# marella/ctransformers

Measured on NVIDIA H100. Metric: decode tokens/s Llama-2-7B Q4_K_M b=1, higher is better.
Workload: dtype int8 (q4_K/q6_K weights x q8_K activations, mma.sync u8 x s8 -> exact int32), fp32 combine in the reference's order

## Files before the change

ctransformers_b200/csrc/matvec.cuh:

```cuda
#pragma once
#include "device_types.cuh"
#include "attention.cuh"

namespace ctb {

#ifndef CTB_THREADS
#define CTB_THREADS 512
#endif
constexpr int MV_THREADS = CTB_THREADS;
constexpr int MV_WARPS = MV_THREADS / 32;
constexpr int MV_ROWS = 4;
constexpr int MV_MAX_SEG = 3;

enum : int { NORM_NONE = 0, NORM_RMS = 1, NORM_LAYER = 2 };
enum : int { EPI_STORE = 0, EPI_ADD = 1, EPI_GELU = 2, EPI_ADD2 = 3, EPI_SILU = 4 };

#ifndef ST_WATCHDOG_NS
#define ST_WATCHDOG_NS 4000000000ull
#endif
#ifndef XC_WATCHDOG_NS
#define XC_WATCHDOG_NS 30000000000ull
#endif
enum WaitCode : int {
  W_GRID_BARRIER = 1, W_FOLD_FLAG, W_FREE_WEIGHT_SLOT, W_WEIGHT_ITEM, W_FREE_K_SLOT, W_FREE_V_SLOT, W_K_ITEM, W_V_ITEM, W_XCHG,
// ... 78 lines not shown

template <bool CG = false>
__device__ __forceinline__ void load16(const float* p, int valid, float (&v)[16]) {
  if (valid >= 16) {
    float4 a, b, c, d;
    if (CG) { a = __ldcg((const float4*)p); b = __ldcg((const float4*)p + 1); c = __ldcg((const float4*)p + 2); d = __ldcg((const float4*)p + 3); }
    else { a = __ldg((const float4*)p); b = __ldg((const float4*)p + 1); c = __ldg((const float4*)p + 2); d = __ldg((const float4*)p + 3); }
    v[0] = a.x; v[1] = a.y; v[2] = a.z; v[3] = a.w; v[4] = b.x; v[5] = b.y; v[6] = b.z; v[7] = b.w;
    v[8] = c.x; v[9] = c.y; v[10] = c.z; v[11] = c.w; v[12] = d.x; v[13] = d.y; v[14] = d.z; v[15] = d.w;
  } else {
#pragma unroll
    for (int e = 0; e < 16; e++) v[e] = e < valid ? (CG ? __ldcg(p + e) : __ldg(p + e)) : 0.f;
  }
}

template <int NT, int BAR>
__device__ __forceinline__ double block_sum_f64(double s, double* red ) {
  s = warp_sum(s);
  bar_sync<BAR, NT>();
  if ((threadIdx.x & 31) == 0) red[threadIdx.x >> 5] = s;
  bar_sync<BAR, NT>();
  double t = 0.0;
#pragma unroll
  for (int w = 0; w < NT / 32; w++) t += red[w];
  return t;
}
template <int NT, int BAR>
__device__ __forceinline__ void block_sum2_max_f64(double& s, double& a, double& g, double* red) {
  constexpr int NW = NT / 32;
#pragma unroll
  for (int o = 16; o > 0; o >>= 1) {
    s += __shfl_xor_sync(0xffffffffu, s, o);
    a += __shfl_xor_sync(0xffffffffu, a, o);
    g = fmax(g, __shfl_xor_sync(0xffffffffu, g, o));
  }
  bar_sync<BAR, NT>();
  if ((threadIdx.x & 31) == 0) { red[threadIdx.x >> 5] = s; red[NW + (threadIdx.x >> 5)] = a; red[2 * NW + (threadIdx.x >> 5)] = g; }
  bar_sync<BAR, NT>();
  s = 0.0;
  a = 0.0;
#pragma unroll
  for (int w = 0; w < NW; w++) { s += red[w]; a += red[NW + w]; g = fmax(g, red[2 * NW + w]); }
}

__device__ __forceinline__ uint32_t pack4(const int* q) {
  return (uint32_t)(q[0] & 0xff) | ((uint32_t)(q[1] & 0xff) << 8) | ((uint32_t)(q[2] & 0xff) << 16) | ((uint32_t)(q[3] & 0xff) << 24);
}

__device__ __forceinline__ void load16_ll(const uint2* p, unsigned epoch, float (&u)[16]) {
  uint4 q[8];
  bounded_wait([&] {
// ... 77 lines not shown
                                           unsigned epoch) {
  const int K = xs.K;
  if (a_is_s) a = s = block_sum_f64<NT, BAR>(s, red);
  else block_sum2_max_f64<NT, BAR>(s, a, g, red);
  if (!isfinite(s) || (!a_is_s && __dmul_ru(a, g) < 0x1p52)) return (float)(s / (double)K);
  const double e = __dmul_ru(a, (double)K * 0x1.0000001p-52);
  const float lo = (float)(__dsub_rd(s, e) / (double)K), hi = (float)(__dadd_ru(s, e) / (double)K);
  if (lo == hi) return lo;
  const double seq = threadIdx.x < 32 ? seq_sum_warp0<XC>(xs.x, xs.x2, xs.x_mode, xs.x_parts, xs.x_stride, K, kind, mean, epoch) : 0.0;
  bar_sync<BAR, NT>();
  if (threadIdx.x == 0) red[0] = seq;
  bar_sync<BAR, NT>();
  return (float)(red[0] / (double)K);
}

template <int NT, int BAR, bool XC = false>
__device__ __forceinline__ void stage_activation(const MVParams& xs, const NormPre& np, int act, uint8_t* smem, double* red, bool write_norm, unsigned epoch = 0) {
  const float* nw = xs.norm_w;
  const float* nb_ = xs.norm_b;
  float* norm_out = xs.norm_out;
  const int norm_mode = xs.norm_mode, K = xs.K;
  const float eps = xs.eps;
  const int t = threadIdx.x, lane = t & 31;
  const int passes = (K + NT * 16 - 1) / (NT * 16);
  float mean = 0.f, scale = 1.f;
  float v0[16];
  load16x<XC>(xs, t * 16, K - t * 16, v0, epoch);
  if (norm_mode == NORM_RMS) {
    double ss = 0.0;
    for (int ps = 0; ps < passes; ps++) {
      const int base = (ps * NT + t) * 16;
      if ((base & ~511) >= K) continue;
// ... 20 lines not shown
        s1 += (double)v[e];
        a1 += (double)fabsf(v[e]);
        emin = min_exp(emin, v[e]);
      }
    }
    mean = norm_stat<NT, BAR, XC>(s1, a1, lsb_inv(emin), false, NORM_TERM_X, 0.f, xs, red, epoch);
    double s2 = 0.0;
    for (int ps = 0; ps < passes; ps++) {
      const int base = (ps * NT + t) * 16;
      if ((base & ~511) >= K) continue;
      float v[16];
      load16x<XC>(xs, base, K - base, v, epoch);
#pragma unroll
      for (int e = 0; e < 16; e++) { const float d = (base + e < K) ? __fsub_rn(v[e], mean) : 0.f; s2 += (double)__fmul_rn(d, d); }
    }
    const float var = norm_stat<NT, BAR, XC>(s2, s2, 0.0, true, NORM_TERM_DEV, mean, xs, red, epoch);
    scale = __fdiv_rn(1.0f, __fsqrt_rn(__fadd_rn(var, eps)));
  }
  int8_t* qs = (int8_t*)smem;
  const size_t off = ((size_t)K + 15) & ~(size_t)15;
  float* dd = (float*)(smem + off);
  int16_t* bs = (int16_t*)(smem + off + q8k_d_bytes(K));
  for (int ps = 0; ps < passes; ps++) {
    const int base = (ps * NT + t) * 16;
    const int valid = K - base;
    if ((base & ~511) >= K) continue;
    float v[16];
    if (ps == 0) {
#pragma unroll
      for (int e = 0; e < 16; e++) v[e] = v0[e];
    } else load16x<XC>(xs, base, valid, v, epoch);
// ... 23 lines not shown
    if (write_norm && norm_out && valid > 0) {
#pragma unroll
      for (int e = 0; e < 16; e++) if (e < valid) norm_out[base + e] = v[e];
    }
    if (act == ACT_Q8_K) {
      float amax = 0.f, mx = 0.f;
#pragma unroll
      for (int e = 0; e < 16; e++) { const float ax = fabsf(v[e]); if (ax > amax) { amax = ax; mx = v[e]; } }
      float gmax = amax;
#pragma unroll
      for (int o = 8; o > 0; o >>= 1) gmax = fmaxf(gmax, __shfl_xor_sync(0xffffffffu, gmax, o));
      const unsigned who = __ballot_sync(0xffffffffu, amax == gmax);
      const int hbase = lane & 16, hl = lane & 15;
      const unsigned mine = (who >> hbase) & 0xffffu;
      const float maxv = __shfl_sync(0xffffffffu, mx, hbase + __ffs(mine) - 1);
      if (valid > 0) {
        const int b = base >> 8;
        int q[16];
        int sum = 0;
        if (gmax == 0.f) {
#pragma unroll
          for (int e = 0; e < 16; e++) q[e] = 0;
          if (hl == 0) dd[b] = 0.f;
        } else {
          const float iscale = __fdiv_rn(-128.f, maxv);
#pragma unroll
          for (int e = 0; e < 16; e++) {
            const float val = __fmaf_rn(iscale, v[e], 12582912.f);
            q[e] = min(127, (__float_as_int(val) & 0x007fffff) - 0x00400000);
            sum += q[e];
          }
          if (hl == 0) dd[b] = __fdiv_rn(1.f, iscale);
        }
        bs[b * 16 + hl] = (int16_t)sum;
#pragma unroll
        for (int j = 0; j < 4; j++) {
          const int wi = hl * 4 + j;
          *(uint32_t*)(qs + q8k_word_offset(b, wi >> 3, wi & 7)) = pack4(q + 4 * j);
        }
      }
    } else if (act == ACT_Q8_0) {
      float amax = 0.f;
#pragma unroll
      for (int e = 0; e < 16; e++) amax = fmaxf(amax, fabsf(v[e]));
      amax = fmaxf(amax, __shfl_xor_sync(0xffffffffu, amax, 1));
      if (valid > 0) {
        const float d = __fdiv_rn(amax, 127.f);
        const float id = amax != 0.f ? __fdiv_rn(127.f, amax) : 0.f;
        int q[16];
#pragma unroll
        for (int e = 0; e < 16; e++) q[e] = __float2int_rn(__fmul_rn(v[e], id));
        *(uint4*)(qs + base) = make_uint4(pack4(q), pack4(q + 4), pack4(q + 8), pack4(q + 12));
        if ((lane & 1) == 0) dd[base >> 5] = h2f(f2h(d));
      }
// ... 156 lines not shown
__device__ __forceinline__ float table_f16(const uint16_t* tab, float x) { return h2f(__ldg(tab + f2h(x))); }

__device__ __forceinline__ float epilogue(int epi, float v, const float* res, const float* res2, const MVParams& p) {
  if (epi == EPI_ADD) return __fadd_rn(v, __ldcg(res));
  if (epi == EPI_ADD2) return __fadd_rn(__fadd_rn(v, __ldcg(res)), __ldcg(res2));
  if (epi == EPI_GELU) return table_f16(p.gelu_tab, v);
  if (epi == EPI_SILU) return table_f16(p.silu_tab, v);
  return v;
}
__device__ __forceinline__ void store_epilogue(const MVSeg& sg, const MVParams& p, int row, float v) { sg.out[row] = epilogue(sg.epi, v, sg.res + row, sg.res2 + row, p); }

__host__ __device__ inline int rows_per_unit(int type) { return (type == GT_F16 || type == GT_F32) ? 1 : MV_ROWS; }

static __global__ void __launch_bounds__(MV_THREADS, 1) k_matvec(const __grid_constant__ MVParams p) {
  extern __shared__ __align__(16) uint8_t smem[];
  __shared__ double red[3 * MV_WARPS];
  const int warp = threadIdx.x >> 5, lane = threadIdx.x & 31;
  pdl_trigger();
  NormPre np;
  preload_norm(np, p);
  pdl_wait();
  stage_activation<MV_THREADS, 0>(p, np, p.act, smem, red, blockIdx.x == 0);
  const ActView a = act_view(p.act, p.K, smem);
  const int gw = blockIdx.x * MV_WARPS + warp, nw = gridDim.x * MV_WARPS;
  int first = gw;
  for (int s = 0; s < p.nseg; s++) {
    const MVSeg& sg = p.seg[s];
    const int type = sg.w.type;
    const int rpu = rows_per_unit(type);
    const int units = (sg.w.M + rpu - 1) / rpu;
    int un = first;
// ... 34 lines not shown
```

ctransformers_b200/csrc/ops_abi.cu:

```cuda
#include <cmath>
#include <cstdio>
#include <cstring>
#include <functional>
#include <memory>
#include <stdexcept>
#include <string>
#include <vector>

#include "../../include/ctransformers_b200.h"
#include "attention.cuh"
#include "matvec.cuh"
#include "prefill.cuh"
#include "repack.cuh"
#include "stream.cuh"
#include "tables.hpp"

using namespace ctb;

namespace {

#define OPS_CUDA(expr)                                                                                     \
  do {                                                                                                     \
    cudaError_t e__ = (expr);                                                                              \
    if (e__ != cudaSuccess) throw std::runtime_error(std::string("CUDA error: ") + cudaGetErrorString(e__) + " (" #expr ")"); \
// ... 69 lines not shown
  o.m.qs = (const uint8_t*)pl[0]; o.m.qh = (const uint8_t*)pl[1]; o.m.d = pl[2]; o.m.mn = pl[3];
}

int sm_count() {
  int n_sm = 132;
  cudaDeviceGetAttribute(&n_sm, cudaDevAttrMultiProcessorCount, 0);
  return n_sm;
}

unsigned* sync_words() {
  static unsigned* d_sync = nullptr;
  if (!d_sync) { OPS_CUDA(cudaMalloc((void**)&d_sync, 64)); OPS_CUDA(cudaMemset(d_sync, 0, 64)); }
  return d_sync;
}

void run_phases(std::vector<Phase> phs) {
  unsigned* d_sync = sync_words();
  const StepLaunch L = step_launch_shape(phs.data(), (int)phs.size(), sm_count(), max_dyn_smem(k_step<true, false>));
  const std::vector<int> hb = step_bounds(phs.data(), (int)phs.size(), L.grid);
  DevBuf dbounds(hb.size() * 4);
  OPS_CUDA(cudaMemcpy(dbounds.p, hb.data(), hb.size() * 4, cudaMemcpyHostToDevice));
  if (L.n_slots < ST_W) throw std::runtime_error("rows too long for the step kernel's shared memory");
  OPS_CUDA(step_set_smem_limit(L.smem));
  DevBuf dprog((phs.size() + 1) * sizeof(Phase));
  OPS_CUDA(cudaMemcpy(dprog.p, phs.data(), phs.size() * sizeof(Phase), cudaMemcpyHostToDevice));
  OPS_CUDA(launch_step(L, 0, dprog.as<Phase>(), dbounds.as<int>(), (int)phs.size(), d_sync));
  OPS_CUDA(cudaGetLastError());
  OPS_CUDA(cudaDeviceSynchronize());
}

void run_matvec(MVParams& p) {
  p.silu_tab = tables().silu;
  p.gelu_tab = tables().gelu;
  if (step_supports(p)) {
    run_phases({matvec_phase(p)});
    return;
  }
  static bool attr = false;
  if (!attr) {
    OPS_CUDA(matvec_set_smem_limit(MV_SMEM_LIMIT));
    attr = true;
  }
  const MVLaunch L = matvec_launch_shape(p, sm_count());
  OPS_CUDA(launch_matvec_kernel(L, 0, p));
  OPS_CUDA(cudaGetLastError());
}

__global__ void __launch_bounds__(MV_THREADS) k_stage_dump(const __grid_constant__ MVParams q, int act, uint8_t* dump) {
  extern __shared__ __align__(16) uint8_t smem[];
  __shared__ double red[3 * MV_WARPS];
  NormPre np;
  preload_norm(np, q);
  stage_activation<MV_THREADS, 0>(q, np, act, smem, red, true);
  const size_t n = act_smem_bytes(act, q.K);
  for (size_t i = threadIdx.x; i < n; i += MV_THREADS) dump[i] = smem[i];
}

__global__ void __launch_bounds__(MV_THREADS) k_gate_dump(const __grid_constant__ MVParams q, float* out) {
  extern __shared__ __align__(16) uint8_t smem[];
  __shared__ double red[3 * MV_WARPS];
  NormPre np;
  preload_norm(np, q);
  stage_activation<MV_THREADS, 0>(q, np, ACT_F32, smem, red, false);
  const float* f = (const float*)smem;
  for (int i = threadIdx.x; i < q.K; i += MV_THREADS) out[i] = f[i];
}

__global__ void k_rope_dump(float* x, const float2* rope, int pos, int hd, int neox) {
  float* row = x + (size_t)blockIdx.x * hd;
  int i0, i1;
  float o0, o1;
  rope_head_pair(row, threadIdx.x, hd, neox, rope[(size_t)pos * (hd / 2) + threadIdx.x], i0, i1, o0, o1);
  row[i0] = o0; row[i1] = o1;
}

int guarded(const char* what, const std::function<void()>& fn) {
  try {
    int ndev = 0;
    if (cudaGetDeviceCount(&ndev) != cudaSuccess || ndev == 0) throw std::runtime_error("no CUDA device available (no CPU fallback)");
    fn();
    return 0;
  } catch (const std::exception& e) {
    fprintf(stderr, "ctransformers-b200: %s failed: %s\n", what, e.what());
    return -1;
  }
}

void stage_to_host(const float* x, const float* w, const float* b, float* y_norm, int mode, float eps, int K, int act, std::vector<uint8_t>& dump) {
  DevBuf dx((size_t)K * 4), dw((size_t)K * 4), db((size_t)K * 4), dy((size_t)K * 4);
  OPS_CUDA(cudaMemcpy(dx.p, x, (size_t)K * 4, cudaMemcpyHostToDevice));
  if (w) OPS_CUDA(cudaMemcpy(dw.p, w, (size_t)K * 4, cudaMemcpyHostToDevice));
  if (b) OPS_CUDA(cudaMemcpy(db.p, b, (size_t)K * 4, cudaMemcpyHostToDevice));
  const size_t n = act_smem_bytes(act, K);
  DevBuf dd(n);
  if (n > 48 * 1024) OPS_CUDA(cudaFuncSetAttribute(k_stage_dump, cudaFuncAttributeMaxDynamicSharedMemorySize, (int)n));
  MVParams q{};
  q.x = dx.as<float>(); q.norm_w = w ? dw.as<float>() : nullptr; q.norm_b = b ? db.as<float>() : nullptr; q.norm_out = dy.as<float>();
  q.norm_mode = mode; q.eps = eps; q.K = K;
  k_stage_dump<<<1, MV_THREADS, n>>>(q, act, dd.as<uint8_t>());
// ... 36 lines not shown
    for (int n = 0; n < N; n++) {
      MVParams p{};
      p.x = dx.as<float>() + (size_t)n * K; p.norm_mode = NORM_NONE; p.K = K; p.act = act_format_for(type); p.nseg = 1;
      p.seg[0].w = w.m; p.seg[0].out = dy.as<float>() + (size_t)n * M; p.seg[0].epi = EPI_STORE;
      run_matvec(p);
    }
    OPS_CUDA(cudaMemcpy(dst, dy.p, (size_t)M * N * 4, cudaMemcpyDeviceToHost));
  });
}

int ctb_quantize_row_q8_K(const float* x, void* y, int k) {
  return guarded("ctb_quantize_row_q8_K", [&] {
    if (k % 256) throw std::runtime_error("k must be a multiple of 256");
    std::vector<uint8_t> dump;
    stage_to_host(x, nullptr, nullptr, nullptr, NORM_NONE, 0.f, k, ACT_Q8_K, dump);
    const int nb = k / 256;
    const size_t off = ((size_t)k + 15) & ~(size_t)15;
    const float* d = (const float*)(dump.data() + off);
    const int16_t* bs = (const int16_t*)(dump.data() + off + q8k_d_bytes(k));
    uint8_t* out = (uint8_t*)y;
    for (int b = 0; b < nb; b++) {
      memcpy(out + (size_t)b * 292, d + b, 4);
      for (int e = 0; e < 256; e++) {
        const int wd = e >> 2, sb = wd >> 3, ln = wd & 7;
        out[(size_t)b * 292 + 4 + e] = dump[(size_t)((b * 2 + (sb >> 2)) * 8 + ln) * 16 + (sb & 3) * 4 + (e & 3)];
      }
      memcpy(out + (size_t)b * 292 + 260, bs + (size_t)b * 16, 32);
    }
  });
}

int ctb_quantize_row_q8_0(const float* x, void* y, int k) {
  return guarded("ctb_quantize_row_q8_0", [&] {
    if (k % 32) throw std::runtime_error("k must be a multiple of 32");
    std::vector<uint8_t> dump;
    stage_to_host(x, nullptr, nullptr, nullptr, NORM_NONE, 0.f, k, ACT_Q8_0, dump);
    const int nb = k / 32;
    const size_t off = ((size_t)k + 15) & ~(size_t)15;
    const float* d = (const float*)(dump.data() + off);
    uint8_t* out = (uint8_t*)y;
    for (int b = 0; b < nb; b++) {
      const uint16_t h = __half_as_ushort(__float2half_rn(d[b]));
      memcpy(out + (size_t)b * 34, &h, 2);
// ... 35 lines not shown
    if (n < 256 || n % 256) throw std::runtime_error("the step kernel takes n a positive multiple of 256");
    const std::vector<uint8_t> zeros(raw_row_bytes(GT_Q4_K, n) * 16, 0);
    OwnedMat wm;
    upload(wm, GT_Q4_K, zeros.data(), n, 16);
    DevBuf dx((size_t)n * 4), dw((size_t)n * 4), db((size_t)n * 4), dy((size_t)n * 4), dout(16 * 4);
    OPS_CUDA(cudaMemcpy(dx.p, x, (size_t)n * 4, cudaMemcpyHostToDevice));
    if (w) OPS_CUDA(cudaMemcpy(dw.p, w, (size_t)n * 4, cudaMemcpyHostToDevice));
    if (b) OPS_CUDA(cudaMemcpy(db.p, b, (size_t)n * 4, cudaMemcpyHostToDevice));
    MVParams p{};
    p.x = dx.as<float>(); p.norm_w = w ? dw.as<float>() : nullptr; p.norm_b = b && mode == NORM_LAYER ? db.as<float>() : nullptr;
    p.norm_out = dy.as<float>(); p.norm_mode = mode; p.eps = eps; p.K = n; p.act = ACT_Q8_K; p.nseg = 1;
    p.seg[0].w = wm.m; p.seg[0].out = dout.as<float>(); p.seg[0].epi = EPI_STORE;
    p.silu_tab = tables().silu; p.gelu_tab = tables().gelu;
    run_phases({matvec_phase(p)});
    OPS_CUDA(cudaMemcpy(y, dy.p, (size_t)n * 4, cudaMemcpyDeviceToHost));
  });
}

int ctb_rope(float* x, int n_heads, int head_dim, int pos, int mode, float freq_base, float freq_scale) {
  return guarded("ctb_rope", [&] {
    const int half = head_dim / 2;
    const std::vector<float2> tab = rope_table(pos + 1, head_dim, head_dim, freq_base, freq_scale);
    const size_t nq = (size_t)n_heads * head_dim;
    DevBuf dq(nq * 4), dtab(tab.size() * 8);
    OPS_CUDA(cudaMemcpy(dq.p, x, nq * 4, cudaMemcpyHostToDevice));
    OPS_CUDA(cudaMemcpy(dtab.p, tab.data(), tab.size() * 8, cudaMemcpyHostToDevice));
    k_rope_dump<<<n_heads, half>>>(dq.as<float>(), dtab.as<float2>(), pos, head_dim, (mode & 2) ? 1 : 0);
    OPS_CUDA(cudaGetLastError());
    OPS_CUDA(cudaMemcpy(x, dq.p, nq * 4, cudaMemcpyDeviceToHost));
  });
// ... 261 lines not shown
```

ctransformers_b200/csrc/prefill.cuh:

```cuda
#pragma once
#include "stream.cuh"

namespace ctb {

constexpr int PB_T = 32;
constexpr int PB_TG = PB_T / 8;
constexpr int PB_TEAMS = 2;
constexpr int PB_W = PB_TEAMS * 4;
constexpr int PB_NT = PB_W * 32;
constexpr int PB_THREADS = PB_NT + 32;
constexpr int PB_BAR = 1;
constexpr int PB_XCH = 12 * 16 * PB_T * 4;

enum : int { PP_EMBED = 0, PP_QUANT = 1, PP_GEMM = 2, PP_KV = 3, PP_ATTN = 4 };

__host__ __device__ inline size_t pb_qbuf_bytes(int K) { return (size_t)(K / 256) * (8192 + 512 + 128); }

struct alignas(16) PPhase {
  int kind;
  MVParams mv;
  int x_ld, x2_ld;
  int out_ld[MV_MAX_SEG], res_ld[MV_MAX_SEG], res2_ld[MV_MAX_SEG];
  uint8_t* qbuf;
  AttnParams at;
// ... 319 lines not shown
__device__ __forceinline__ void pb_attn_phase(const PPhase& ph, int n_tok, uint8_t* work) {
  const int warp = threadIdx.x >> 5;
  const int n_tasks = n_tok * ph.at.n_head;
  uint8_t* wsm = work + (size_t)warp * pb_attn_warp_bytes(ph.at.n_ctx, ph.at.hd);
  for (int task = blockIdx.x * PB_W + warp; task < n_tasks; task += (int)gridDim.x * PB_W) {
    const int tok = task / ph.at.n_head;
    pb_attn_warp_task<GEN>(ph.at, ph.state + tok * 4, tok, task % ph.at.n_head, wsm);
  }
}
static __device__ __noinline__ void pb_attn_phase_gen(const PPhase& ph, int n_tok, uint8_t* work) { pb_attn_phase<true>(ph, n_tok, work); }

static __global__ void __launch_bounds__(PB_THREADS, 1) k_pstep(const __grid_constant__ PStepArgs args) {
  extern __shared__ __align__(16) uint8_t smem[];
  __shared__ __align__(8) uint64_t full_bar[ST_MAX_SLOTS];
  __shared__ __align__(8) uint64_t empty_bar[ST_MAX_SLOTS];
  __shared__ double red[3 * PB_W];
  __shared__ __align__(16) PPhase ph;
  const int warp = threadIdx.x >> 5;
  uint8_t* ring = smem;
  uint8_t* work = smem + (size_t)args.n_slots * ST_SLOT;
  ring_init(full_bar, empty_bar, args.n_slots, 4);
  if (warp == PB_W) {
    pb_producer(args, ring, full_bar, empty_bar);
    return;
  }
  const unsigned G = gridDim.x;
  uint32_t seq = 0;
#pragma unroll 1
  for (int ip = 0; ip < args.n_phases; ip++) {
    bar_sync<PB_BAR, PB_NT>();
    if (threadIdx.x == 0 && ip > 0) { __threadfence(); atomicAdd(args.sync, 1u); }
// ... 76 lines not shown
```

ctransformers_b200/csrc/stream.cuh:

```cuda
#pragma once
#include "matvec.cuh"

namespace ctb {

#ifndef CTB_ST_WARPS
#define CTB_ST_WARPS 10
#endif
constexpr int ST_W = CTB_ST_WARPS;
constexpr int ST_NT = ST_W * 32;
constexpr int ST_THREADS = ST_NT + 32;
constexpr int ST_SLOT = 9216;
#ifndef CTB_ST_DEPTH
#define CTB_ST_DEPTH 2
#endif
constexpr int ST_MAX_DEPTH = CTB_ST_DEPTH;
constexpr int ST_MAX_SLOTS = ST_W * ST_MAX_DEPTH;
constexpr int ST_MAXT = 16;
constexpr int ST_ROWS = 16;
constexpr int ST_BAR = 1;
constexpr int ST_STATE = 6;

#ifndef CTB_CHUNK_Q4
#define CTB_CHUNK_Q4 4
#endif
// ... 104 lines not shown
  asm("mma.sync.aligned.m16n8k32.row.col.s32.u8.s8.s32 {%0,%1,%2,%3}, {%4,%5,%6,%7}, {%8,%9}, {%10,%11,%12,%13};"
      : "=r"(d[0]), "=r"(d[1]), "=r"(d[2]), "=r"(d[3])
      : "r"(a0), "r"(a1), "r"(a2), "r"(a3), "r"(b0), "r"(b1), "r"(c0), "r"(c1), "r"(c0), "r"(c1));
}

struct StAct {
  const int8_t* qs;
  const float* d;
  const uint32_t* pairs;
  const int* cneg;
  const int8_t* zero;
  const struct XchgParams* xc;
  unsigned epoch;
};
__host__ __device__ inline size_t st_off_pairs(int K) { return ((((size_t)K + 15) & ~(size_t)15) + q8k_d_bytes(K) + (size_t)(K / 16) * 2 + 15) & ~(size_t)15; }
__host__ __device__ inline size_t st_act_bytes(int K, bool q6) { return st_off_pairs(K) + (size_t)(K / 256) * 16 + (q6 ? (size_t)K : 0) + 256 + 16; }

template <int NT, int BAR>
__device__ __forceinline__ StAct st_act_extras(uint8_t* smem, int K, bool q6) {
  const ActView a = act_view(ACT_Q8_K, K, smem);
  StAct s;
  s.qs = a.qs; s.d = a.d;
  uint32_t* pairs = (uint32_t*)(smem + st_off_pairs(K));
  int* cneg = (int*)(smem + st_off_pairs(K) + (size_t)(K / 256) * 16);
  s.pairs = pairs; s.cneg = cneg;
  const int nb = K >> 8;
  int* zero = (int*)(smem + st_off_pairs(K) + (size_t)nb * 16 + (q6 ? (size_t)K : 0));
  s.zero = (const int8_t*)zero;
  if (threadIdx.x < 64) zero[threadIdx.x] = 0;
  for (int i = threadIdx.x; i < nb * 4; i += NT) {
    const int16_t* b4 = a.bs + (i >> 2) * 16 + 4 * (i & 3);
    const int p0 = (int)b4[0] + (int)b4[1], p1 = (int)b4[2] + (int)b4[3];
    pairs[i] = (uint32_t)(p0 & 0xffff) | ((uint32_t)p1 << 16);
  }
  if (q6) {
    for (int i = threadIdx.x; i < nb * 64; i += NT) {
      const int b = i >> 6, grp = (i >> 3) & 7, l = i & 7;
      const int w = *(const int*)(a.qs + q8k_word_offset(b, grp, l));
      cneg[((b * 4 + (l >> 1)) * 8 + grp) * 2 + (l & 1)] = -32 * __dp4a(0x01010101, w, 0);
    }
  }
  bar_sync<BAR, NT>();
  return s;
}

__device__ __forceinline__ void unpack_k4(uint32_t s0, uint32_t s1, uint32_t s2, uint32_t& sc03, uint32_t& sc47, uint32_t& m03, uint32_t& m47) {
  sc03 = s0 & 0x3f3f3f3fu;
  m03 = s1 & 0x3f3f3f3fu;
  sc47 = (s2 & 0x0f0f0f0fu) | (((s0 >> 6) & 0x03030303u) << 4);
  m47 = ((s2 >> 4) & 0x0f0f0f0fu) | (((s1 >> 6) & 0x03030303u) << 4);
}
__device__ __forceinline__ int pack16(int lo, int hi) { return (int)__byte_perm((uint32_t)lo, (uint32_t)hi, 0x5410); }
__device__ __forceinline__ int scale_fold8(int d0, int d1, int d2, int d3, int d4, int d5, int d6, int d7, uint32_t s03, uint32_t s47) {
  int s = __dp2a_lo(pack16(d0, d1), (int)s03, 0);
  s = __dp2a_hi(pack16(d2, d3), (int)s03, s);
  s = __dp2a_lo(pack16(d4, d5), (int)s47, s);
  s = __dp2a_hi(pack16(d6, d7), (int)s47, s);
// ... 279 lines not shown
  int q6;
  MVParams mv;
  AttnParams at;
  EmbedParams em;
  PickParams pk;
  XchgParams xc;
};

struct StepArgs {
  const Phase* prog;
  int n_phases;
  int n_slots;
  unsigned* sync;
  const int* bounds;
  unsigned long long* trace;
};

__device__ __forceinline__ unsigned ld_relaxed_u32(const unsigned* p) {
  unsigned v;
  asm volatile("ld.relaxed.gpu.global.u32 %0, [%1];" : "=r"(v) : "l"(p) : "memory");
  return v;
}
__device__ __forceinline__ unsigned ld_acquire_u32(const unsigned* p) {
  unsigned v;
  asm volatile("ld.acquire.gpu.global.u32 %0, [%1];" : "=r"(v) : "l"(p) : "memory");
  return v;
}

struct TileInfo { int seg, til, nch, type; };
__device__ __forceinline__ TileInfo tile_info(const TileSpace& ts, const MVParams& p, int tile, int nb, bool valid) {
// ... 175 lines not shown
            mbar_expect_tx(&full_bar[rp.slot], it.bytes);
            bulk_g2s_hint(ring + (size_t)rp.slot * ST_SLOT, it.src, it.bytes, &full_bar[rp.slot], weight_pol);
          }
          __syncwarp();
        }
        __syncwarp();
        seq += (uint32_t)__popc(mask);
      }
    }
  }
}

template <bool XC>
__device__ __forceinline__ void st_matvec_phase(const Phase& ph, const NormPre& np, uint8_t* ring, uint8_t* act_smem, double* red, uint64_t* full_bar, uint64_t* empty_bar,
                                                float (*mailbox)[ST_STATE * 32], int* flags, uint32_t S, uint32_t& seq, const int* tb, unsigned long long* tr,
                                                unsigned xc_base) {
  const MVParams& p = ph.mv;
  const int warp = threadIdx.x >> 5, lane = threadIdx.x & 31;
  const unsigned epoch = XC ? xc_base + (unsigned)ph.xc.index + 1u : 0u;
  stage_activation<ST_NT, ST_BAR, XC>(p, np, ACT_Q8_K, act_smem, red, blockIdx.x == 0, epoch);
  StAct a = st_act_extras<ST_NT, ST_BAR>(act_smem, p.K, ph.q6 != 0);
  a.xc = XC && ph.xc.role == 2 ? &ph.xc : nullptr;
  a.epoch = epoch;
  if (tr && threadIdx.x == 0) tr[1] = globaltimer_ns();
  bool first_item = tr != nullptr && threadIdx.x == 0;
  TileSpace ts;
  ts.init(p);
  const int nb = p.K >> 8;
  const int T0 = tb[0], T1 = tb[1];
#pragma unroll 1
  for (int w0 = T0; w0 < T1; w0 += ST_MAXT) {
    if (w0 != T0) {
      bar_sync<ST_BAR, ST_NT>();
      if (threadIdx.x < ST_MAXT) flags[threadIdx.x] = 0;
      bar_sync<ST_BAR, ST_NT>();
    }
    const int ntw = min(ST_MAXT, T1 - w0);
    const TileInfo ti = tile_info(ts, p, w0 + lane, nb, lane < ntw);
#pragma unroll 1
// ... 43 lines not shown
    __threadfence();
    if (atomicAdd(sync + 1, 1u) == gridDim.x - 1) {
      sync[0] = 0u;
      sync[1] = 0u;
      if (set_xc) sync[2] = xc;
      __threadfence();
    }
  }
}

template <bool XC, bool GEN>
static __global__ void __launch_bounds__(ST_THREADS, 1) k_step(const __grid_constant__ StepArgs args) {
  extern __shared__ __align__(16) uint8_t smem[];
  __shared__ __align__(8) uint64_t full_bar[ST_MAX_SLOTS];
  __shared__ __align__(8) uint64_t empty_bar[ST_MAX_SLOTS];
  __shared__ double red[3 * ST_W];
  __shared__ __align__(16) float mailbox[ST_MAXT][ST_STATE * 32];
  __shared__ int flags[ST_MAXT];
  __shared__ float pick_v[ST_W];
  __shared__ int pick_i[ST_W];
  __shared__ __align__(16) Phase ph_s[2];
  __shared__ int tb_s[2][2];
  const int warp = threadIdx.x >> 5;
  uint8_t* ring = smem;
  uint8_t* act_smem = smem + (size_t)args.n_slots * ST_SLOT;
  ring_init(full_bar, empty_bar, args.n_slots, 1);
  pdl_trigger();
  pdl_wait();
  if (warp == ST_W) {
    st_producer<XC, GEN>(args, ring, full_bar, empty_bar);
    return;
  }
  const unsigned G = gridDim.x;
  uint32_t seq = 0;
  const unsigned xc_base = XC ? ld_relaxed_u32(args.sync + 2) : 0u;
  unsigned xc_done = 0;
  auto fetch_phase = [&](int ip) {
    if (ip >= args.n_phases) return;
    const uint4* src = (const uint4*)(args.prog + ip);
    const uint32_t dst = st_smem(&ph_s[ip & 1]);
    const int i = (int)threadIdx.x - 32;
    if (i >= 0 && i < (int)(sizeof(Phase) / 16)) asm volatile("cp.async.ca.shared.global [%0], [%1], 16;" ::"r"(dst + i * 16), "l"(src + i) : "memory");
    if (i >= 64 && i < 66)
      asm volatile("cp.async.ca.shared.global [%0], [%1], 4;" ::"r"(st_smem(&tb_s[ip & 1][i - 64])), "l"(args.bounds + (size_t)ip * (gridDim.x + 1) + blockIdx.x + (i - 64)) : "memory");
    asm volatile("cp.async.commit_group;" ::: "memory");
  };
  fetch_phase(0);
#pragma unroll 1
  for (int ip = 0; ip < args.n_phases; ip++) {
    bar_sync<ST_BAR, ST_NT>();
    unsigned long long* const tr = args.trace ? args.trace + ((size_t)ip * G + blockIdx.x) * 8 : nullptr;
    if (tr && threadIdx.x == 0) tr[4] = globaltimer_ns();
    if (threadIdx.x == 0 && ip > 0) {
      const unsigned target = (unsigned)ip * G;
      asm volatile("red.release.gpu.global.add.u32 [%0], 1;" ::"l"(args.sync) : "memory");
      if (tr) tr[5] = globaltimer_ns();
      bounded_wait([&] { return ld_relaxed_u32(args.sync) >= target; }, W_GRID_BARRIER, ip);
      if (tr) { tr[6] = globaltimer_ns(); tr[7] = tr[6]; }
    } else {
      asm volatile("cp.async.wait_all;" ::: "memory");
      if (threadIdx.x >= 32 && threadIdx.x < 32 + ST_MAXT) flags[threadIdx.x - 32] = 0;
    }
    bar_sync<ST_BAR, ST_NT>();
    const Phase& ph = ph_s[ip & 1];
    fetch_phase(ip + 1);
    NormPre np;
    if (ph.kind == PH_MATVEC) preload_norm(np, ph.mv);
    if (tr && threadIdx.x == 0) tr[0] = globaltimer_ns();
    if (XC && ph.kind == PH_MATVEC && ph.xc.role == 1) xc_done++;
    if (ph.kind == PH_MATVEC) {
      st_matvec_phase<XC>(ph, np, ring, act_smem, red, full_bar, empty_bar, mailbox, flags, (uint32_t)(args.n_slots / ST_W), seq, &tb_s[ip & 1][0], tr, xc_base);
    } else if (ph.kind == PH_ATTN) {
      if (GEN) seq = st_attn_phase_gen(ph, act_smem, ring, full_bar, empty_bar, args.n_slots, seq, pick_v, red);
      else st_attn_phase<false>(ph, act_smem, ring, full_bar, empty_bar, args.n_slots, seq, pick_v, red);
    } else if (ph.kind == PH_EMBED) {
      if (blockIdx.x == 0) embed_row(ph.em, ph.em.tokens[0], ph.em.out, threadIdx.x, ST_NT);
    } else if (ph.kind == PH_PICK) {
      if (blockIdx.x == 0) st_pick_phase(ph.pk, pick_v, pick_i);
    }
    if (tr) {
      bar_sync<ST_BAR, ST_NT>();
      if (threadIdx.x == 0) tr[3] = globaltimer_ns();
    }
  }
  bar_sync<ST_BAR, ST_NT>();
  grid_rearm(args.sync, XC, xc_base + xc_done);
// ... 43 lines not shown
  ph.kind = PH_MATVEC;
  ph.mv = p;
  ph.mv.act = ACT_Q8_K;
  for (int s = 0; s < p.nseg; s++) ph.q6 |= p.seg[s].w.type == GT_Q6_K;
  return ph;
}

static inline cudaError_t st_set_debug_words(int* dev_ptr) { return cudaMemcpyToSymbol(g_st_dbg, &dev_ptr, sizeof(int*)); }
static inline cudaError_t step_set_smem_limit(size_t bytes) {
  cudaError_t e = cudaFuncSetAttribute(k_step<false, false>, cudaFuncAttributeMaxDynamicSharedMemorySize, (int)bytes);
  if (e == cudaSuccess) e = cudaFuncSetAttribute(k_step<false, true>, cudaFuncAttributeMaxDynamicSharedMemorySize, (int)bytes);
  return e != cudaSuccess ? e : cudaFuncSetAttribute(k_step<true, false>, cudaFuncAttributeMaxDynamicSharedMemorySize, (int)bytes);
}

static inline cudaError_t launch_step(const StepLaunch& L, cudaStream_t st, const Phase* d_prog, const int* d_bounds, int n_phases, unsigned* d_sync, bool pdl = false,
                                      unsigned long long* trace = nullptr, bool xchg = false) {
  StepArgs a;
  a.prog = d_prog; a.bounds = d_bounds; a.n_phases = n_phases; a.n_slots = L.n_slots; a.sync = d_sync; a.trace = trace;
  return launch_kernel(xchg ? k_step<true, false> : (L.gen ? k_step<false, true> : k_step<false, false>), dim3(L.grid), dim3(ST_THREADS), L.smem, st, pdl, a);
}

}
```

ctransformers_b200/lib.py:

```python
import ctypes as C
from pathlib import Path
from typing import Optional

LIB_DIR = Path(__file__).resolve().parent / "lib"
LIB_NAME = "libctransformers.so"


class ConfigStruct(C.Structure):
    _fields_ = [("context_length", C.c_int), ("gpu_layers", C.c_int), ("mmap", C.c_bool), ("mlock", C.c_bool)]


def find_library(path: Optional[str] = None) -> str:
    if path:
        return str(path)
    lib = LIB_DIR / LIB_NAME
    if not lib.is_file():
        raise OSError(
            f"{lib} has not been built. Build it with `python -m ctransformers_b200.build` "
            "(needs nvcc; compiles for sm_90a). There is no CPU fallback library."
        )
    return str(lib)


_P = C.c_void_p
# ... 30 lines not shown
    "ctb_llm_device_samples": (C.c_long, [_P]),
    "ctb_llm_set_stream": (None, [_P, C.c_void_p]),
    "ctb_tp_unique_id": (C.c_int, [_P, C.c_int]),
    "ctb_llm_create_tp": (_P, [C.c_char_p, C.c_char_p, ConfigStruct, C.c_int, C.c_int, _P]),
    "ctb_tp_shard": (C.c_int, [C.c_int, C.c_int, C.c_int, C.c_int, C.c_int, C.c_int, _IP]),
    "ctb_llm_decode_greedy": (C.c_double, [_P, C.c_int, C.c_int, C.c_int, _IP]),
    "ctb_llm_profile_step": (C.c_int, [_P, C.c_int, C.c_int, C.POINTER(C.c_double), _IP]),
    "ctb_llm_time_matvec_only": (C.c_double, [_P, C.c_int, C.POINTER(C.c_long)]),
    "ctb_llm_time_matvec_kinds": (C.c_double, [_P, C.c_int, C.POINTER(C.c_long), C.c_uint]),
    "ctb_mul_mat": (C.c_int, [C.c_int, _P, _P, _P, C.c_int, C.c_int, C.c_int]),
    "ctb_quantize_row_q8_K": (C.c_int, [_P, _P, C.c_int]),
    "ctb_quantize_row_q8_0": (C.c_int, [_P, _P, C.c_int]),
    "ctb_quantize_row_q8_1": (C.c_int, [_P, _P, C.c_int]),
    "ctb_norm": (C.c_int, [C.c_int, _P, _P, _P, _P, C.c_int, C.c_float]),
    "ctb_norm_path": (C.c_int, [C.c_int, C.c_int, _P, _P, _P, _P, C.c_int, C.c_float]),
    "ctb_rope": (C.c_int, [_P, C.c_int, C.c_int, C.c_int, C.c_int, C.c_float, C.c_float]),
    "ctb_attention": (C.c_int, [_P, _P, _P, _P, C.c_int, C.c_int, C.c_int, C.c_int, C.c_int, C.c_float]),
    "ctb_attention_path": (C.c_int, [C.c_int, _P, _P, _P, _P, _P, _P, C.c_int, C.c_int, C.c_int, C.c_int, C.c_int, C.c_int, _P, C.c_int,
                                     C.c_float, C.c_float]),
    "ctb_prefill_mul_mat": (C.c_int, [C.c_int, _P, _P, _P, C.c_int, C.c_int, _P, _P, C.c_int, _P, _P, C.c_float, _P, _P, _P, _P, C.c_int,
                                      C.c_int, _P]),
    "ctb_llm_paths": (C.c_long, [_P, _IP, C.c_int]),
    "ctb_ffn_gate": (C.c_int, [C.c_int, _P, _P, _P, _P, C.c_int, C.c_int]),
    "ctb_matvec_partition": (C.c_int, [_IP, _IP, C.c_int, C.c_int, C.c_int, _IP, _IP]),
    "ctb_get_row": (C.c_int, [C.c_int, _P, C.c_int, C.c_int, C.c_int, _P]),
    "ctb_vocab_load": (_P, [C.c_char_p]),
    "ctb_vocab_free": (None, [_P]),
    "ctb_vocab_size": (C.c_int, [_P]),
    "ctb_vocab_tokenize": (C.c_int, [_P, C.c_char_p, C.c_bool, _IP, C.c_int]),
    "ctb_vocab_piece": (C.c_int, [_P, C.c_int, C.c_char_p, C.c_int]),
# ... 17 lines not shown
```

include/ctransformers_b200.h:

```cpp
#ifndef CTRANSFORMERS_B200_H_
#define CTRANSFORMERS_B200_H_

#include <stdbool.h>
#include <stddef.h>
#include <stdint.h>

#ifdef __cplusplus
extern "C" {
#endif

typedef struct LLM LLM;

typedef struct ctransformers_config {
  int context_length;
  int gpu_layers;
  bool mmap;
  bool mlock;
} ctransformers_config;

LLM* ctransformers_llm_create(const char* model_path, const char* model_type, const ctransformers_config config);
void ctransformers_llm_delete(LLM* llm);
int ctransformers_llm_tokenize(LLM* llm, const char* text, const bool add_bos_token, int* output);
const char* ctransformers_llm_detokenize(LLM* llm, const int token);
bool ctransformers_llm_is_eos_token(LLM* llm, const int token);
// ... 35 lines not shown
typedef struct ctb_vocab ctb_vocab;
ctb_vocab* ctb_vocab_load(const char* gguf_path);
void ctb_vocab_free(ctb_vocab* v);
int ctb_vocab_size(ctb_vocab* v);
int ctb_vocab_tokenize(ctb_vocab* v, const char* text, bool add_bos, int* out, int cap);
int ctb_vocab_piece(ctb_vocab* v, int token, char* buf, int cap);
int ctb_sample(const float* logits, int n_vocab, const int* last_tokens, int n_last, int top_k, float top_p, float temperature,
               float repetition_penalty, int seed);

int ctb_mul_mat(int type, const void* w_blocks, const float* x, float* dst, int K, int M, int N);
int ctb_quantize_row_q8_K(const float* x, void* y, int k);
int ctb_quantize_row_q8_0(const float* x, void* y, int k);
int ctb_quantize_row_q8_1(const float* x, void* y, int k);
int ctb_norm(int mode, const float* x, const float* w, const float* b, float* y, int n, float eps);
int ctb_norm_path(int path, int mode, const float* x, const float* w, const float* b, float* y, int n, float eps);
int ctb_rope(float* x, int n_heads, int head_dim, int pos, int mode, float freq_base, float freq_scale);
int ctb_attention(const float* q, const uint16_t* kcache, const uint16_t* vcache, float* out, int n_head, int n_kv, int head_dim,
                  int T, int n_total, float kq_scale);
int ctb_attention_path(int path, const float* q, const float* k_new, const float* v_new, uint16_t* kcache, uint16_t* vcache,
                       float* out, int n_head, int n_kv, int head_dim, int n_ctx, int pos0, int n_tok, const int* n_total,
                       int rope_mode, float freq_base, float kq_scale);
int ctb_prefill_mul_mat(int nseg, const int* types, const void* const* w_blocks, const int* rows, int K, int n_tok, const float* x,
                        const float* x2, int norm_mode, const float* norm_w, const float* norm_b, float eps, const int* epi,
                        const float* res, const float* res2, float* out, int n_ctx, int head_dim, int* n_slots);
int ctb_ffn_gate(int type, const void* w1_blocks, const void* w3_blocks, const float* x, float* out, int K, int M);
int ctb_matvec_partition(const int* types, const int* rows, int nseg, int K, int n_sm, int* first_tile, int* meta);

int ctb_get_row(int type, const void* table_blocks, int K, int n_rows, int row, float* out);

#ifdef __cplusplus
// ... 4 lines not shown
```

Before: 365.6.

## Fuse Q8_K pair sums and Q6 cneg into activation staging, trim barriers

```diff
diff --git a/ctransformers_b200/csrc/matvec.cuh b/ctransformers_b200/csrc/matvec.cuh
--- a/ctransformers_b200/csrc/matvec.cuh
+++ b/ctransformers_b200/csrc/matvec.cuh
@@ -116,10 +116,11 @@
   }
 }
 
+template <int NT> constexpr int stage_red_doubles() { return 4 * (NT / 32); }
+
 template <int NT, int BAR>
 __device__ __forceinline__ double block_sum_f64(double s, double* red ) {
   s = warp_sum(s);
-  bar_sync<BAR, NT>();
   if ((threadIdx.x & 31) == 0) red[threadIdx.x >> 5] = s;
   bar_sync<BAR, NT>();
   double t = 0.0;
@@ -136,7 +137,6 @@
     a += __shfl_xor_sync(0xffffffffu, a, o);
     g = fmax(g, __shfl_xor_sync(0xffffffffu, g, o));
   }
-  bar_sync<BAR, NT>();
   if ((threadIdx.x & 31) == 0) { red[threadIdx.x >> 5] = s; red[NW + (threadIdx.x >> 5)] = a; red[2 * NW + (threadIdx.x >> 5)] = g; }
   bar_sync<BAR, NT>();
   s = 0.0;
@@ -244,8 +244,14 @@
   return (float)(red[0] / (double)K);
 }
 
+struct Q8KExtras {
+  uint32_t* pairs = nullptr;
+  int* cneg = nullptr;
+};
+
 template <int NT, int BAR, bool XC = false>
-__device__ __forceinline__ void stage_activation(const MVParams& xs, const NormPre& np, int act, uint8_t* smem, double* red, bool write_norm, unsigned epoch = 0) {
+__device__ __forceinline__ void stage_activation(const MVParams& xs, const NormPre& np, int act, uint8_t* smem, double* red, bool write_norm, unsigned epoch = 0,
+                                                 Q8KExtras ex = {}) {
   const float* nw = xs.norm_w;
   const float* nb_ = xs.norm_b;
   float* norm_out = xs.norm_out;
@@ -296,7 +302,7 @@
 #pragma unroll
       for (int e = 0; e < 16; e++) { const float d = (base + e < K) ? __fsub_rn(v[e], mean) : 0.f; s2 += (double)__fmul_rn(d, d); }
     }
-    const float var = norm_stat<NT, BAR, XC>(s2, s2, 0.0, true, NORM_TERM_DEV, mean, xs, red, epoch);
+    const float var = norm_stat<NT, BAR, XC>(s2, s2, 0.0, true, NORM_TERM_DEV, mean, xs, red + 3 * (NT / 32), epoch);
     scale = __fdiv_rn(1.0f, __fsqrt_rn(__fadd_rn(var, eps)));
   }
   int8_t* qs = (int8_t*)smem;
@@ -350,10 +356,10 @@
       const int hbase = lane & 16, hl = lane & 15;
       const unsigned mine = (who >> hbase) & 0xffffu;
       const float maxv = __shfl_sync(0xffffffffu, mx, hbase + __ffs(mine) - 1);
+      const int b = base >> 8;
+      int sum = 0;
       if (valid > 0) {
-        const int b = base >> 8;
         int q[16];
-        int sum = 0;
         if (gmax == 0.f) {
 #pragma unroll
           for (int e = 0; e < 16; e++) q[e] = 0;
@@ -369,11 +375,23 @@
           if (hl == 0) dd[b] = __fdiv_rn(1.f, iscale);
         }
         bs[b * 16 + hl] = (int16_t)sum;
+        uint32_t w[4];
 #pragma unroll
         for (int j = 0; j < 4; j++) {
           const int wi = hl * 4 + j;
-          *(uint32_t*)(qs + q8k_word_offset(b, wi >> 3, wi & 7)) = pack4(q + 4 * j);
+          w[j] = pack4(q + 4 * j);
+          *(uint32_t*)(qs + q8k_word_offset(b, wi >> 3, wi & 7)) = w[j];
         }
+        if (ex.cneg) {
+          int* c = ex.cneg + ((b * 4 + (hl & 1) * 2) * 8 + (hl >> 1)) * 2;
+          *(int2*)c = make_int2(-32 * __dp4a(0x01010101, (int)w[0], 0), -32 * __dp4a(0x01010101, (int)w[1], 0));
+          *(int2*)(c + 16) = make_int2(-32 * __dp4a(0x01010101, (int)w[2], 0), -32 * __dp4a(0x01010101, (int)w[3], 0));
+        }
+      }
+      if (ex.pairs) {
+        const int s01 = sum + __shfl_down_sync(0xffffffffu, sum, 1);
+        const int s23 = __shfl_down_sync(0xffffffffu, s01, 2);
+        if (valid > 0 && (hl & 3) == 0) ex.pairs[b * 4 + (hl >> 2)] = (uint32_t)(s01 & 0xffff) | ((uint32_t)s23 << 16);
       }
     } else if (act == ACT_Q8_0) {
       float amax = 0.f;
@@ -560,7 +578,7 @@
 
 static __global__ void __launch_bounds__(MV_THREADS, 1) k_matvec(const __grid_constant__ MVParams p) {
   extern __shared__ __align__(16) uint8_t smem[];
-  __shared__ double red[3 * MV_WARPS];
+  __shared__ double red[stage_red_doubles<MV_THREADS>()];
   const int warp = threadIdx.x >> 5, lane = threadIdx.x & 31;
   pdl_trigger();
   NormPre np;
diff --git a/ctransformers_b200/csrc/ops_abi.cu b/ctransformers_b200/csrc/ops_abi.cu
--- a/ctransformers_b200/csrc/ops_abi.cu
+++ b/ctransformers_b200/csrc/ops_abi.cu
@@ -107,7 +107,7 @@
   return d_sync;
 }
 
-void run_phases(std::vector<Phase> phs) {
+void run_phases(std::vector<Phase> phs, uint8_t* act_dump = nullptr) {
   unsigned* d_sync = sync_words();
   const StepLaunch L = step_launch_shape(phs.data(), (int)phs.size(), sm_count(), max_dyn_smem(k_step<true, false>));
   const std::vector<int> hb = step_bounds(phs.data(), (int)phs.size(), L.grid);
@@ -117,7 +117,7 @@
   OPS_CUDA(step_set_smem_limit(L.smem));
   DevBuf dprog((phs.size() + 1) * sizeof(Phase));
   OPS_CUDA(cudaMemcpy(dprog.p, phs.data(), phs.size() * sizeof(Phase), cudaMemcpyHostToDevice));
-  OPS_CUDA(launch_step(L, 0, dprog.as<Phase>(), dbounds.as<int>(), (int)phs.size(), d_sync));
+  OPS_CUDA(launch_step(L, 0, dprog.as<Phase>(), dbounds.as<int>(), (int)phs.size(), d_sync, false, nullptr, false, act_dump));
   OPS_CUDA(cudaGetLastError());
   OPS_CUDA(cudaDeviceSynchronize());
 }
@@ -141,7 +141,7 @@
 
 __global__ void __launch_bounds__(MV_THREADS) k_stage_dump(const __grid_constant__ MVParams q, int act, uint8_t* dump) {
   extern __shared__ __align__(16) uint8_t smem[];
-  __shared__ double red[3 * MV_WARPS];
+  __shared__ double red[stage_red_doubles<MV_THREADS>()];
   NormPre np;
   preload_norm(np, q);
   stage_activation<MV_THREADS, 0>(q, np, act, smem, red, true);
@@ -151,7 +151,7 @@
 
 __global__ void __launch_bounds__(MV_THREADS) k_gate_dump(const __grid_constant__ MVParams q, float* out) {
   extern __shared__ __align__(16) uint8_t smem[];
-  __shared__ double red[3 * MV_WARPS];
+  __shared__ double red[stage_red_doubles<MV_THREADS>()];
   NormPre np;
   preload_norm(np, q);
   stage_activation<MV_THREADS, 0>(q, np, ACT_F32, smem, red, false);
@@ -176,6 +176,20 @@
   } catch (const std::exception& e) {
     fprintf(stderr, "ctransformers-b200: %s failed: %s\n", what, e.what());
     return -1;
+  }
+}
+
+void q8k_image_to_blocks(const uint8_t* img, int k, uint8_t* out) {
+  const size_t off = ((size_t)k + 15) & ~(size_t)15;
+  const float* d = (const float*)(img + off);
+  const int16_t* bs = (const int16_t*)(img + off + q8k_d_bytes(k));
+  for (int b = 0; b < k / 256; b++) {
+    memcpy(out + (size_t)b * 292, d + b, 4);
+    for (int e = 0; e < 256; e++) {
+      const int wd = e >> 2, sb = wd >> 3, ln = wd & 7;
+      out[(size_t)b * 292 + 4 + e] = img[(size_t)((b * 2 + (sb >> 2)) * 8 + ln) * 16 + (sb & 3) * 4 + (e & 3)];
+    }
+    memcpy(out + (size_t)b * 292 + 260, bs + (size_t)b * 16, 32);
   }
 }
 
@@ -242,19 +256,7 @@
     if (k % 256) throw std::runtime_error("k must be a multiple of 256");
     std::vector<uint8_t> dump;
     stage_to_host(x, nullptr, nullptr, nullptr, NORM_NONE, 0.f, k, ACT_Q8_K, dump);
-    const int nb = k / 256;
-    const size_t off = ((size_t)k + 15) & ~(size_t)15;
-    const float* d = (const float*)(dump.data() + off);
-    const int16_t* bs = (const int16_t*)(dump.data() + off + q8k_d_bytes(k));
-    uint8_t* out = (uint8_t*)y;
-    for (int b = 0; b < nb; b++) {
-      memcpy(out + (size_t)b * 292, d + b, 4);
-      for (int e = 0; e < 256; e++) {
-        const int wd = e >> 2, sb = wd >> 3, ln = wd & 7;
-        out[(size_t)b * 292 + 4 + e] = dump[(size_t)((b * 2 + (sb >> 2)) * 8 + ln) * 16 + (sb & 3) * 4 + (e & 3)];
-      }
-      memcpy(out + (size_t)b * 292 + 260, bs + (size_t)b * 16, 32);
-    }
+    q8k_image_to_blocks(dump.data(), k, (uint8_t*)y);
   });
 }
 
@@ -320,6 +322,47 @@
     p.silu_tab = tables().silu; p.gelu_tab = tables().gelu;
     run_phases({matvec_phase(p)});
     OPS_CUDA(cudaMemcpy(y, dy.p, (size_t)n * 4, cudaMemcpyDeviceToHost));
+  });
+}
+
+int ctb_step_stage(int K, const float* x, const float* x2, int norm_mode, const float* norm_w, const float* norm_b, float eps, int nseg,
+                   const int* types, void* q8k, uint32_t* pairs, int32_t* cneg) {
+  return guarded("ctb_step_stage", [&] {
+    if (K < 256 || K % 256) throw std::runtime_error("K must be a positive multiple of 256");
+    if (nseg < 1 || nseg > MV_MAX_SEG) throw std::runtime_error("1 to 3 segments");
+    if (norm_mode < NORM_NONE || norm_mode > NORM_LAYER) throw std::runtime_error("norm mode 0, 1 or 2");
+    if (norm_mode != NORM_NONE && !norm_w) throw std::runtime_error("a norm needs norm_w");
+    bool q6 = false;
+    for (int s = 0; s < nseg; s++) {
+      if (!type_is_kquant(types[s])) throw std::runtime_error("the step kernel takes K-quant weights only");
+      q6 |= types[s] == GT_Q6_K;
+    }
+    if (q6 && !cneg) throw std::runtime_error("a Q6_K segment needs cneg");
+    std::unique_ptr<OwnedMat> mats[MV_MAX_SEG];
+    DevBuf dx((size_t)K * 4), dx2((size_t)K * 4), dw((size_t)K * 4), db((size_t)K * 4), dout((size_t)MV_MAX_SEG * 16 * 4);
+    MVParams p{};
+    for (int s = 0; s < nseg; s++) {
+      const std::vector<uint8_t> zeros(raw_row_bytes(types[s], K) * 16, 0);
+      mats[s].reset(new OwnedMat());
+      upload(*mats[s], types[s], zeros.data(), K, 16);
+      p.seg[s].w = mats[s]->m; p.seg[s].out = dout.as<float>() + s * 16; p.seg[s].epi = EPI_STORE;
+    }
+    OPS_CUDA(cudaMemcpy(dx.p, x, (size_t)K * 4, cudaMemcpyHostToDevice));
+    if (x2) OPS_CUDA(cudaMemcpy(dx2.p, x2, (size_t)K * 4, cudaMemcpyHostToDevice));
+    if (norm_w) OPS_CUDA(cudaMemcpy(dw.p, norm_w, (size_t)K * 4, cudaMemcpyHostToDevice));
+    if (norm_b) OPS_CUDA(cudaMemcpy(db.p, norm_b, (size_t)K * 4, cudaMemcpyHostToDevice));
+    p.x = dx.as<float>(); p.x2 = x2 ? dx2.as<float>() : nullptr; p.x_mode = x2 ? 1 : 0;
+    p.norm_w = norm_mode != NORM_NONE ? dw.as<float>() : nullptr; p.norm_b = norm_mode == NORM_LAYER && norm_b ? db.as<float>() : nullptr;
+    p.norm_mode = norm_mode; p.eps = eps; p.K = K; p.act = ACT_Q8_K; p.nseg = nseg;
+    p.silu_tab = tables().silu; p.gelu_tab = tables().gelu;
+    const size_t n = st_act_bytes(K, q6);
+    DevBuf dimg(n);
+    run_phases({matvec_phase(p)}, dimg.as<uint8_t>());
+    std::vector<uint8_t> img(n);
+    OPS_CUDA(cudaMemcpy(img.data(), dimg.p, n, cudaMemcpyDeviceToHost));
+    q8k_image_to_blocks(img.data(), K, (uint8_t*)q8k);
+    memcpy(pairs, img.data() + st_off_pairs(K), (size_t)(K / 256) * 16);
+    if (q6) memcpy(cneg, img.data() + st_off_pairs(K) + (size_t)(K / 256) * 16, (size_t)K);
   });
 }
 
diff --git a/ctransformers_b200/csrc/prefill.cuh b/ctransformers_b200/csrc/prefill.cuh
--- a/ctransformers_b200/csrc/prefill.cuh
+++ b/ctransformers_b200/csrc/prefill.cuh
@@ -357,7 +357,7 @@
   extern __shared__ __align__(16) uint8_t smem[];
   __shared__ __align__(8) uint64_t full_bar[ST_MAX_SLOTS];
   __shared__ __align__(8) uint64_t empty_bar[ST_MAX_SLOTS];
-  __shared__ double red[3 * PB_W];
+  __shared__ double red[stage_red_doubles<PB_NT>()];
   __shared__ __align__(16) PPhase ph;
   const int warp = threadIdx.x >> 5;
   uint8_t* ring = smem;
diff --git a/ctransformers_b200/csrc/stream.cuh b/ctransformers_b200/csrc/stream.cuh
--- a/ctransformers_b200/csrc/stream.cuh
+++ b/ctransformers_b200/csrc/stream.cuh
@@ -142,33 +142,18 @@
   unsigned epoch;
 };
 __host__ __device__ inline size_t st_off_pairs(int K) { return ((((size_t)K + 15) & ~(size_t)15) + q8k_d_bytes(K) + (size_t)(K / 16) * 2 + 15) & ~(size_t)15; }
-__host__ __device__ inline size_t st_act_bytes(int K, bool q6) { return st_off_pairs(K) + (size_t)(K / 256) * 16 + (q6 ? (size_t)K : 0) + 256 + 16; }
-
-template <int NT, int BAR>
-__device__ __forceinline__ StAct st_act_extras(uint8_t* smem, int K, bool q6) {
+__host__ __device__ inline size_t st_act_bytes(int K, bool q6) { return st_off_pairs(K) + (size_t)(K / 256) * 16 + (q6 ? (size_t)K : 0) + 16; }
+
+__device__ __forceinline__ Q8KExtras st_extras(uint8_t* smem, int K, bool q6) {
+  Q8KExtras e;
+  e.pairs = (uint32_t*)(smem + st_off_pairs(K));
+  e.cneg = q6 ? (int*)(smem + st_off_pairs(K) + (size_t)(K / 256) * 16) : nullptr;
+  return e;
+}
+__device__ __forceinline__ StAct st_act_view(uint8_t* smem, int K, const Q8KExtras& e, const int8_t* zero) {
   const ActView a = act_view(ACT_Q8_K, K, smem);
   StAct s;
-  s.qs = a.qs; s.d = a.d;
-  uint32_t* pairs = (uint32_t*)(smem + st_off_pairs(K));
-  int* cneg = (int*)(smem + st_off_pairs(K) + (size_t)(K / 256) * 16);
-  s.pairs = pairs; s.cneg = cneg;
-  const int nb = K >> 8;
-  int* zero = (int*)(smem + st_off_pairs(K) + (size_t)nb * 16 + (q6 ? (size_t)K : 0));
-  s.zero = (const int8_t*)zero;
-  if (threadIdx.x < 64) zero[threadIdx.x] = 0;
-  for (int i = threadIdx.x; i < nb * 4; i += NT) {
-    const int16_t* b4 = a.bs + (i >> 2) * 16 + 4 * (i & 3);
-    const int p0 = (int)b4[0] + (int)b4[1], p1 = (int)b4[2] + (int)b4[3];
-    pairs[i] = (uint32_t)(p0 & 0xffff) | ((uint32_t)p1 << 16);
-  }
-  if (q6) {
-    for (int i = threadIdx.x; i < nb * 64; i += NT) {
-      const int b = i >> 6, grp = (i >> 3) & 7, l = i & 7;
-      const int w = *(const int*)(a.qs + q8k_word_offset(b, grp, l));
-      cneg[((b * 4 + (l >> 1)) * 8 + grp) * 2 + (l & 1)] = -32 * __dp4a(0x01010101, w, 0);
-    }
-  }
-  bar_sync<BAR, NT>();
+  s.qs = a.qs; s.d = a.d; s.pairs = e.pairs; s.cneg = e.cneg; s.zero = zero;
   return s;
 }
 
@@ -478,6 +463,7 @@
   unsigned* sync;
   const int* bounds;
   unsigned long long* trace;
+  uint8_t* act_dump;
 };
 
 __device__ __forceinline__ unsigned ld_relaxed_u32(const unsigned* p) {
@@ -683,15 +669,18 @@
 template <bool XC>
 __device__ __forceinline__ void st_matvec_phase(const Phase& ph, const NormPre& np, uint8_t* ring, uint8_t* act_smem, double* red, uint64_t* full_bar, uint64_t* empty_bar,
                                                 float (*mailbox)[ST_STATE * 32], int* flags, uint32_t S, uint32_t& seq, const int* tb, unsigned long long* tr,
-                                                unsigned xc_base) {
+                                                unsigned xc_base, const int8_t* zero, uint8_t* act_dump) {
   const MVParams& p = ph.mv;
   const int warp = threadIdx.x >> 5, lane = threadIdx.x & 31;
   const unsigned epoch = XC ? xc_base + (unsigned)ph.xc.index + 1u : 0u;
-  stage_activation<ST_NT, ST_BAR, XC>(p, np, ACT_Q8_K, act_smem, red, blockIdx.x == 0, epoch);
-  StAct a = st_act_extras<ST_NT, ST_BAR>(act_smem, p.K, ph.q6 != 0);
+  const Q8KExtras ex = st_extras(act_smem, p.K, ph.q6 != 0);
+  stage_activation<ST_NT, ST_BAR, XC>(p, np, ACT_Q8_K, act_smem, red, blockIdx.x == 0, epoch, ex);
+  StAct a = st_act_view(act_smem, p.K, ex, zero);
   a.xc = XC && ph.xc.role == 2 ? &ph.xc : nullptr;
   a.epoch = epoch;
   if (tr && threadIdx.x == 0) tr[1] = globaltimer_ns();
+  if (act_dump && blockIdx.x == 0)
+    for (int i = threadIdx.x; i < (int)(st_act_bytes(p.K, ph.q6 != 0) / 16); i += ST_NT) ((uint4*)act_dump)[i] = ((const uint4*)act_smem)[i];
   bool first_item = tr != nullptr && threadIdx.x == 0;
   TileSpace ts;
   ts.init(p);
@@ -765,7 +754,8 @@
   extern __shared__ __align__(16) uint8_t smem[];
   __shared__ __align__(8) uint64_t full_bar[ST_MAX_SLOTS];
   __shared__ __align__(8) uint64_t empty_bar[ST_MAX_SLOTS];
-  __shared__ double red[3 * ST_W];
+  __shared__ double red[stage_red_doubles<ST_NT>()];
+  __shared__ __align__(16) int zero_run[64];
   __shared__ __align__(16) float mailbox[ST_MAXT][ST_STATE * 32];
   __shared__ int flags[ST_MAXT];
   __shared__ float pick_v[ST_W];
@@ -775,6 +765,7 @@
   const int warp = threadIdx.x >> 5;
   uint8_t* ring = smem;
   uint8_t* act_smem = smem + (size_t)args.n_slots * ST_SLOT;
+  if (threadIdx.x < 64) zero_run[threadIdx.x] = 0;
   ring_init(full_bar, empty_bar, args.n_slots, 1);
   pdl_trigger();
   pdl_wait();
@@ -799,28 +790,29 @@
   fetch_phase(0);
 #pragma unroll 1
   for (int ip = 0; ip < args.n_phases; ip++) {
+    asm volatile("cp.async.wait_all;" ::: "memory");
     bar_sync<ST_BAR, ST_NT>();
     unsigned long long* const tr = args.trace ? args.trace + ((size_t)ip * G + blockIdx.x) * 8 : nullptr;
     if (tr && threadIdx.x == 0) tr[4] = globaltimer_ns();
+    const Phase& ph = ph_s[ip & 1];
     if (threadIdx.x == 0 && ip > 0) {
       const unsigned target = (unsigned)ip * G;
       asm volatile("red.release.gpu.global.add.u32 [%0], 1;" ::"l"(args.sync) : "memory");
       if (tr) tr[5] = globaltimer_ns();
       bounded_wait([&] { return ld_relaxed_u32(args.sync) >= target; }, W_GRID_BARRIER, ip);
       if (tr) { tr[6] = globaltimer_ns(); tr[7] = tr[6]; }
-    } else {
-      asm volatile("cp.async.wait_all;" ::: "memory");
-      if (threadIdx.x >= 32 && threadIdx.x < 32 + ST_MAXT) flags[threadIdx.x - 32] = 0;
-    }
-    bar_sync<ST_BAR, ST_NT>();
-    const Phase& ph = ph_s[ip & 1];
-    fetch_phase(ip + 1);
+    } else if (threadIdx.x >= 32 && threadIdx.x < 32 + ST_MAXT) {
+      flags[threadIdx.x - 32] = 0;
+    }
     NormPre np;
     if (ph.kind == PH_MATVEC) preload_norm(np, ph.mv);
+    bar_sync<ST_BAR, ST_NT>();
+    fetch_phase(ip + 1);
     if (tr && threadIdx.x == 0) tr[0] = globaltimer_ns();
     if (XC && ph.kind == PH_MATVEC && ph.xc.role == 1) xc_done++;
     if (ph.kind == PH_MATVEC) {
-      st_matvec_phase<XC>(ph, np, ring, act_smem, red, full_bar, empty_bar, mailbox, flags, (uint32_t)(args.n_slots / ST_W), seq, &tb_s[ip & 1][0], tr, xc_base);
+      st_matvec_phase<XC>(ph, np, ring, act_smem, red, full_bar, empty_bar, mailbox, flags, (uint32_t)(args.n_slots / ST_W), seq, &tb_s[ip & 1][0], tr, xc_base,
+                          (const int8_t*)zero_run, args.act_dump);
     } else if (ph.kind == PH_ATTN) {
       if (GEN) seq = st_attn_phase_gen(ph, act_smem, ring, full_bar, empty_bar, args.n_slots, seq, pick_v, red);
       else st_attn_phase<false>(ph, act_smem, ring, full_bar, empty_bar, args.n_slots, seq, pick_v, red);
@@ -894,9 +886,9 @@
 }
 
 static inline cudaError_t launch_step(const StepLaunch& L, cudaStream_t st, const Phase* d_prog, const int* d_bounds, int n_phases, unsigned* d_sync, bool pdl = false,
-                                      unsigned long long* trace = nullptr, bool xchg = false) {
+                                      unsigned long long* trace = nullptr, bool xchg = false, uint8_t* act_dump = nullptr) {
   StepArgs a;
-  a.prog = d_prog; a.bounds = d_bounds; a.n_phases = n_phases; a.n_slots = L.n_slots; a.sync = d_sync; a.trace = trace;
+  a.prog = d_prog; a.bounds = d_bounds; a.n_phases = n_phases; a.n_slots = L.n_slots; a.sync = d_sync; a.trace = trace; a.act_dump = act_dump;
   return launch_kernel(xchg ? k_step<true, false> : (L.gen ? k_step<false, true> : k_step<false, false>), dim3(L.grid), dim3(ST_THREADS), L.smem, st, pdl, a);
 }
 
diff --git a/ctransformers_b200/lib.py b/ctransformers_b200/lib.py
--- a/ctransformers_b200/lib.py
+++ b/ctransformers_b200/lib.py
@@ -68,6 +68,7 @@
     "ctb_quantize_row_q8_1": (C.c_int, [_P, _P, C.c_int]),
     "ctb_norm": (C.c_int, [C.c_int, _P, _P, _P, _P, C.c_int, C.c_float]),
     "ctb_norm_path": (C.c_int, [C.c_int, C.c_int, _P, _P, _P, _P, C.c_int, C.c_float]),
+    "ctb_step_stage": (C.c_int, [C.c_int, _P, _P, C.c_int, _P, _P, C.c_float, C.c_int, _P, _P, _P, _P]),
     "ctb_rope": (C.c_int, [_P, C.c_int, C.c_int, C.c_int, C.c_int, C.c_float, C.c_float]),
     "ctb_attention": (C.c_int, [_P, _P, _P, _P, C.c_int, C.c_int, C.c_int, C.c_int, C.c_int, C.c_float]),
     "ctb_attention_path": (C.c_int, [C.c_int, _P, _P, _P, _P, _P, _P, C.c_int, C.c_int, C.c_int, C.c_int, C.c_int, C.c_int, _P, C.c_int,
diff --git a/include/ctransformers_b200.h b/include/ctransformers_b200.h
--- a/include/ctransformers_b200.h
+++ b/include/ctransformers_b200.h
@@ -73,6 +73,8 @@
 int ctb_quantize_row_q8_1(const float* x, void* y, int k);
 int ctb_norm(int mode, const float* x, const float* w, const float* b, float* y, int n, float eps);
 int ctb_norm_path(int path, int mode, const float* x, const float* w, const float* b, float* y, int n, float eps);
+int ctb_step_stage(int K, const float* x, const float* x2, int norm_mode, const float* norm_w, const float* norm_b, float eps, int nseg,
+                   const int* types, void* q8k, uint32_t* pairs, int32_t* cneg);
 int ctb_rope(float* x, int n_heads, int head_dim, int pos, int mode, float freq_base, float freq_scale);
 int ctb_attention(const float* q, const uint16_t* kcache, const uint16_t* vcache, float* out, int n_head, int n_kv, int head_dim,
                   int T, int n_total, float kq_scale);
```

Measured after the change: 369.6 (median of 6 runs). 1.1% higher.
